# mattreturn1/ComputerVision_ObjectDetection_FeatureMatching

Hardware: AMD Instinct MI355X
Metric: matches+homographies/sec (10k x 10k SIFT, 50k RANSAC iters) at 1/2/4/8 GPUs (higher is better)
Workload: dtype i8-MFMA exact-int distances (i32 acc), fp64 DLT/Jacobi, fp32 reprojection; 1 GPU; c4: one global batch of 256 scenes x 1 model set, 10000x10000 descriptors, maxIters 50000, scenes sharded over 1 GPU(s) (256 on rank 0); problems_per_gpu=256, global_batch=256, parallelism=dp1, batches_in_flight=16, dist_backend=nccl, hw_queues=24

## Files before the change

computervision_objectdetection_featurematching_amd/csrc/api.cpp:

```cpp
#include <hip/hip_runtime.h>

#include <algorithm>
#include <cfloat>
#include <climits>
#include <cmath>
#include <cstdarg>
#include <cstdio>
#include <cstdlib>
#include <cstring>
#include <map>
#include <mutex>
#include <string>
#include <vector>

#include "../../include/mim.h"
#include "../../include/mim_detect.hpp"
#include "knn_coll.h"
#include "mim_internal.h"
#include "radius.h"

namespace mim {
void launch_prep_batch(const PrepJob* jobs, int njobs, int total_tiles, hipStream_t st);
void launch_knn(const ProbDev* probs, const KnnWork* works, int n_works, const int* seg_start, int n_blocks, Top2* parts,
                int* dyn_ctr, float kappa, float flip_ratio, hipStream_t st);
// ... 134 lines not shown
            if (p[i]) (void)hipHostFree(p[i]);
            if (ev[i]) (void)hipEventDestroy(ev[i]);
            p[i] = nullptr;
            ev[i] = nullptr;
        }
    }
};

template <class T> size_t vec_bytes(const std::vector<T>& v) { return sizeof(T) * v.size(); }

struct StageWriter {
    PinnedStage& ps;
    hipStream_t s;
    char* p = nullptr;
    size_t off = 0;
    hipError_t err;
    StageWriter(PinnedStage& ps_, size_t total, hipStream_t s_) : ps(ps_), s(s_) { err = ps.acquire(total, &p); }
    void put(void* dst, const void* a, size_t ab, const void* b = nullptr, size_t bb = 0) {
        if (err != hipSuccess || ab + bb == 0) return;
        if (ab) memcpy(p + off, a, ab);
        if (bb) memcpy(p + off + ab, b, bb);
        err = hipMemcpyAsync(dst, p + off, ab + bb, hipMemcpyHostToDevice, s);
        off += ab + bb;
    }
    template <class T> void put(const DevBuf& dst, const std::vector<T>& v) { put(dst.p, v.data(), vec_bytes(v)); }
    hipError_t done() { return err != hipSuccess ? err : ps.release_after(s); }
};

}

namespace mim {
struct RansacWs {
    DevBuf state, samples, hyp, counts, bounds, flags, irr_bits, irr, irr_cnt, cls, cls_tab, pass_bits, defer, defer_n, chains, best_h, cand, ncand, cex, cH, decided, stream,
        scratch, inl, tiles, tbox, perm, surv, nsurv, err;
    long long stream_len = 0;
};
}

struct mim_ctx {
    int device = 0;
    hipStream_t own = nullptr, stream = nullptr;
    std::mutex mu;
    std::string err;
    Arena arena;
    std::vector<SetRec> sets;
    DevBuf probs, works, parts, good_q, good_t, pts, n_good, results, masks, knn_idx, knn_dist, inl_tab, inl_out, knn_ctr, ham_works, flt_works;
    RansacWs rws;
    std::vector<ProbDev> h_probs;
    int n_ham_works = 0;
    int n_flt_works = 0;
    DevBuf ham_cross_works, colmin, cross_tab;
    int n_ham_cross_works = 0;
    long long n_colmin = 0;
    DevBuf topk_parts, topk_ham_works, topk_flt_works, topk_probs;
    int topk_splits = 0;
    DevBuf coll_parts, coll_ham_works, coll_flt_works, coll_i8_probs, coll_i8_works, coll_tab, coll_queries;
    int coll_groups = 0;
    int coll_i8_splits = 0;
    DevBuf rad_counts, rad_cursor, rad_offsets, rad_meta, rad_keys, rad_scratch, rad_ham_works, rad_flt_works, rad_i8_works,
        rad_probs;
    struct RadLast {
        bool valid = false;
        std::vector<mim_problem> problems;
        float r = 0.f;
        long long gen = -1;
        long long n_queries = 0, total = 0, longest = 0;
        int n_ham = 0, n_flt = 0, n_i8_works = 0, n_i8_blocks = 0;
// ... 105 lines not shown
    }
    c->stream = c->own;
    c->cur = c->own;
    const char* ex = getenv("MIM_RANSAC_EXACT");
    c->exact_all = (ex && ex[0] == '1') ? 1 : 0;
    const char* cc = getenv("MIM_CAND_CAP");
    c->cand_cap = cc ? std::max(1, atoi(cc)) : 0;
    const char* rc = getenv("MIM_ATTEMPT_REP_CAP");
    c->rep_cap = rc ? std::max(1, atoi(rc)) : 0;
    const char* sd = getenv("MIM_STREAM_DRAWS");
    c->stream_draws = sd ? std::max(4096LL, atoll(sd)) : 0;
    *out = c;
    return MIM_OK;
}

void mim_ctx_destroy(mim_ctx* c) {
    if (!c) return;
    (void)hipSetDevice(c->device);
    (void)hipStreamSynchronize(c->stream);
    for (auto& e : c->evs) (void)hipEventDestroy(e.e);
    for (hipEvent_t e : c->ev_pool) (void)hipEventDestroy(e);
    if (c->samp) (void)hipStreamSynchronize(c->samp);
    if (c->ev_samp_fork) (void)hipEventDestroy(c->ev_samp_fork);
    for (auto e : c->ev_samp)
        if (e) (void)hipEventDestroy(e);
    if (c->samp) (void)hipStreamDestroy(c->samp);
    mim::sift_ws_destroy(c->sift);
    for (mim::SiftWs* w : c->sift_scales) mim::sift_ws_destroy(w);
    c->stage.destroy();
    c->prep_stage.destroy();
    c->arena.release();
    for (DevBuf* b : {&c->probs, &c->works, &c->parts, &c->good_q, &c->good_t, &c->pts, &c->n_good,
                      &c->results, &c->masks, &c->knn_idx, &c->knn_dist, &c->inl_tab, &c->inl_out, &c->knn_ctr, &c->ham_works, &c->flt_works, &c->ham_cross_works, &c->colmin, &c->cross_tab, &c->topk_parts, &c->topk_ham_works, &c->topk_flt_works, &c->topk_probs, &c->coll_parts, &c->coll_ham_works, &c->coll_flt_works, &c->coll_i8_probs, &c->coll_i8_works, &c->coll_tab, &c->coll_queries, &c->rad_counts, &c->rad_cursor, &c->rad_offsets, &c->rad_meta, &c->rad_keys, &c->rad_scratch, &c->rad_ham_works, &c->rad_flt_works, &c->rad_i8_works, &c->rad_probs, &c->rws.state, &c->rws.samples,
                      &c->rws.hyp, &c->rws.counts, &c->rws.bounds, &c->rws.flags, &c->rws.irr_bits, &c->rws.irr, &c->rws.irr_cnt, &c->rws.cls, &c->rws.cls_tab, &c->rws.pass_bits, &c->rws.defer, &c->rws.defer_n, &c->rws.chains, &c->rws.best_h, &c->rws.cand, &c->rws.ncand, &c->rws.cex, &c->rws.cH, &c->rws.decided, &c->rws.stream, &c->rws.scratch, &c->rws.inl, &c->rws.tiles, &c->rws.tbox, &c->rws.perm, &c->rws.surv, &c->rws.nsurv, &c->rws.err, &c->prep_jobs})
        b->release();
    if (c->own) (void)hipStreamDestroy(c->own);
    delete c;
}

const char* mim_last_error(const mim_ctx* c) { return c ? c->err.c_str() : "null ctx"; }

mim_status mim_ctx_set_stream(mim_ctx* c, void* stream) {
    if (!c) return MIM_EINVAL;
    std::lock_guard<std::mutex> lk(c->mu);
    c->stream = stream ? (hipStream_t)stream : c->own;
    return MIM_OK;
}

mim_status mim_ctx_set_sampler_stream(mim_ctx* c, int32_t on) {
    if (!c) return MIM_EINVAL;
    std::lock_guard<std::mutex> lk(c->mu);
    c->samp_on = on != 0;
    return MIM_OK;
}

void* mim_ctx_get_stream(const mim_ctx* c) { return c ? (void*)c->stream : nullptr; }

mim_status mim_synchronize(mim_ctx* c) {
    if (!c) return MIM_EINVAL;
    HIPCHK(c, hipSetDevice(c->device));
    HIPCHK(c, hipStreamSynchronize(c->stream));
    return MIM_OK;
}

mim_status mim_set_timing(mim_ctx* c, int32_t enable) {
    if (!c) return MIM_EINVAL;
    c->timing = enable != 0;
// ... 1517 lines not shown
    }
    HIPCHK(c, c->rws.state.ensure(sizeof(RansacState) * std::max(n, 1)));
    HIPCHK(c, c->rws.samples.ensure(sizeof(int4) * it_total));
    HIPCHK(c, c->rws.hyp.ensure(sizeof(float) * 8 * it_total));
    HIPCHK(c, c->rws.counts.ensure(sizeof(int) * it_total));
    HIPCHK(c, c->rws.bounds.ensure(sizeof(int2) * it_total));
    const long long chunk_max = std::min<long long>(max_iters, 1 << 18);
    flag_per = (chunk_max * 28 + 4096 + 63) & ~63LL;
    const long long flag_cap = (long long)std::max(n, 1) * flag_per;
    HIPCHK(c, c->rws.flags.ensure((size_t)flag_cap));
    HIPCHK(c, c->rws.irr_bits.ensure((size_t)flag_cap / 8));
    const int irr_blocks = (int)((flag_per + kIrrBlock - 1) / kIrrBlock);
    HIPCHK(c, c->rws.irr.ensure(sizeof(int) * (size_t)std::max(n, 1) * irr_blocks * kIrrCap));
    HIPCHK(c, c->rws.irr_cnt.ensure(sizeof(int) * (size_t)std::max(n, 1) * irr_blocks));
    HIPCHK(c, c->rws.cls.ensure(sizeof(SamplerClass) * (size_t)std::max(n, 1)));
    HIPCHK(c, c->rws.cls_tab.ensure(sizeof(SamplerClassSlot) * ((size_t)q_max + 1)));
    HIPCHK(c, c->rws.pass_bits.ensure((size_t)flag_cap / 8));
    const int def_rounds = (int)((flag_per / 4 + 2 * kRansacDefRoundAttempts) / kRansacDefRoundAttempts);
    HIPCHK(c, c->rws.defer.ensure(sizeof(int2) * kRansacDefSlots * (size_t)std::max(n, 1) * def_rounds));
    HIPCHK(c, c->rws.defer_n.ensure(sizeof(int) * (size_t)std::max(n, 1) * def_rounds));
    HIPCHK(c, c->rws.chains.ensure(ransac_chain_bytes() * (size_t)std::max(n, 1)));
    HIPCHK(c, c->rws.best_h.ensure(sizeof(double) * 9 * std::max(n, 1)));
    const size_t cap = (size_t)std::max(n, 1) * 2 * kCandPerProblem;
    HIPCHK(c, c->rws.cand.ensure(sizeof(int) * cap));
    HIPCHK(c, c->rws.ncand.ensure(sizeof(int) * 2 * std::max(n, 1)));
    HIPCHK(c, c->rws.cex.ensure(sizeof(int) * cap));
    HIPCHK(c, c->rws.cH.ensure(sizeof(double) * 9 * cap));
    HIPCHK(c, c->rws.decided.ensure(sizeof(int) * cap));
    HIPCHK(c, c->rws.inl.ensure(sizeof(float4) * good_total));
    HIPCHK(c, c->rws.tiles.ensure(sizeof(uint4) * 128 * ((good_total + 31) / 32)));
    HIPCHK(c, c->rws.tbox.ensure(sizeof(float4) * ((good_total + 31) / 32)));
    HIPCHK(c, c->rws.perm.ensure(sizeof(int) * 2 * good_total));
    HIPCHK(c, c->rws.surv.ensure(sizeof(int) * it_total));
    HIPCHK(c, c->rws.nsurv.ensure(sizeof(int) * std::max(n, 1)));
    HIPCHK(c, c->rws.err.ensure(sizeof(int) * 4));
    HIPCHK(c, c->results.ensure(sizeof(mim_result) * std::max(n, 1)));
    HIPCHK(c, c->masks.ensure(good_total));
    HIPCHK(c, hipMemsetAsync(c->rws.err.p, 0, sizeof(int) * 4, c->stream));
    b = RansacBufs{};
    b.state = c->rws.state.as<RansacState>();
    b.samples = c->rws.samples.as<int4>();
    b.hyp = c->rws.hyp.as<float>();
    b.counts = c->rws.counts.as<int>();
    b.bounds = c->rws.bounds.as<int2>();
    b.flags = c->rws.flags.as<uint8_t>();
    b.irr_bits = c->rws.irr_bits.as<uint8_t>();
    b.best_h = c->rws.best_h.as<double>();
    b.cand = c->rws.cand.as<int>();
    b.ncand = c->rws.ncand.as<int>();
    b.cex = c->rws.cex.as<int>();
    b.cH = c->rws.cH.as<double>();
    b.decided = c->rws.decided.as<int>();
    b.flag_cap = flag_cap;
    b.irr = c->rws.irr.as<int>();
    b.irr_cnt = c->rws.irr_cnt.as<int>();
    b.pass_bits = c->rws.pass_bits.as<uint32_t>();
    b.defer = c->rws.defer.as<int2>();
    b.defer_n = c->rws.defer_n.as<int>();
    const char* cde = getenv("MIM_CHECK_DEFER");
    b.def_rounds = (cde && cde[0] == '0') ? 0 : def_rounds;
    b.irr_blocks = irr_blocks;
    b.cls = c->rws.cls.as<SamplerClass>();
    b.cls_tab = c->rws.cls_tab.as<SamplerClassSlot>();
    b.cls_tab_n = q_max + 1;
    b.chains = c->rws.chains.p;
    b.stream = c->rws.stream.as<uint32_t>();
    b.stream_len = c->rws.stream_len;
    b.inl = c->rws.inl.as<float4>();
    b.tiles = c->rws.tiles.as<uint4>();
    b.tbox = c->rws.tbox.as<float4>();
    b.perm = c->rws.perm.as<int>();
    b.surv = c->rws.surv.as<int>();
    b.nsurv = c->rws.nsurv.as<int>();
    b.err = c->rws.err.as<int>();
    if (c->samp_on < 0) {
        const char* e = getenv("MIM_SAMPLER_STREAM");
        c->samp_on = (e && e[0] == '0') ? 0 : 1;
    }
    if (c->samp_on && !c->samp) {
        HIPCHK(c, hipStreamCreateWithFlags(&c->samp, hipStreamNonBlocking));
        HIPCHK(c, hipEventCreateWithFlags(&c->ev_samp_fork, hipEventDisableTiming));
        for (auto& e : c->ev_samp) HIPCHK(c, hipEventCreateWithFlags(&e, hipEventDisableTiming));
    }
    b.s2 = c->samp_on ? c->samp : nullptr;
    b.ev_fork = c->ev_samp_fork;
    b.ev_samp[0] = c->ev_samp[0];
    b.ev_samp[1] = c->ev_samp[1];
    rp = RansacParams{};
    rp.thresh = prm->ransac_thresh > 0 ? prm->ransac_thresh : 3.0;
    rp.conf = prm->confidence;
    rp.max_iters = max_iters;
    rp.ratio = prm->ratio;
    rp.min_good = prm->min_good;
    rp.min_inliers = prm->min_inliers;
    rp.det_lo = prm->det_lo;
    rp.det_hi = prm->det_hi;
    rp.cand_cap = c->cand_cap;
    rp.rep_cap = c->rep_cap;
    return MIM_OK;
}

static mim_status ransac_enqueue_range(mim_ctx* c, int p0, int np, const RansacBufs& b, const RansacParams& rp,
                                       long long flag_per, int raw) {
    RansacBufs g = b;
    g.state += p0;
    g.flags += (long long)p0 * flag_per;
    g.irr_bits += (long long)p0 * flag_per / 8;
    g.flag_cap = (long long)np * flag_per;
    g.irr += (long long)p0 * b.irr_blocks * kIrrCap;
    g.irr_cnt += (long long)p0 * b.irr_blocks;
    g.cls += p0;
    g.pass_bits += (long long)p0 * flag_per / 32;
    g.defer += (long long)p0 * b.def_rounds * kRansacDefSlots;
    g.defer_n += (long long)p0 * b.def_rounds;
    g.chains = static_cast<char*>(b.chains) + (size_t)p0 * ransac_chain_bytes();
    g.best_h += 9LL * p0;
    g.cand += (long long)p0 * 2 * kCandPerProblem;
    g.ncand += 2 * p0;
    g.cex += (long long)p0 * 2 * kCandPerProblem;
    g.cH += 9LL * p0 * 2 * kCandPerProblem;
    g.decided += (long long)p0 * 2 * kCandPerProblem;
    g.nsurv += p0;
    ransac_enqueue(rp, np, c->probs.as<ProbDev>() + p0, c->pts.as<float4>(), c->n_good.as<int>() + p0, g,
                   c->masks.as<uint8_t>(), c->results.as<mim_result>() + p0, raw, c->cur, mark_cb, c, c->exact_all);
    HIPCHK(c, hipGetLastError());
    return MIM_OK;
}

static mim_status ransac_locked(mim_ctx* c, int n, const mim_params* prm, int raw) {
    RansacBufs b;
    RansacParams rp;
    long long flag_per = 0;
    mim_status s = ransac_prepare(c, n, prm, b, rp, flag_per);
    if (s != MIM_OK) return s;
    c->cur = c->stream;
    return ransac_enqueue_range(c, 0, n, b, rp, flag_per, raw);
}

static mim_status check_params(mim_ctx* c, const mim_params* p) {
    if (!p) return fail(c, MIM_EINVAL, "null params");
    if (!(p->confidence > 0 && p->confidence < 1)) return fail(c, MIM_EINVAL, "confidence must be in (0,1)");
    if (p->max_iters > 10000000) return fail(c, MIM_EINVAL, "max_iters too large");
    return MIM_OK;
}

extern "C" {

}

static mim_status batch_run_locked(mim_ctx* c, const mim_problem* problems, int32_t n, const mim_params* params,
                                   int filter) {
    HIPCHK(c, hipSetDevice(c->device));
    c->last_problems.assign(problems, problems + n);
    c->last_params = *params;
    c->last_filter = filter;
// ... 225 lines not shown
```

computervision_objectdetection_featurematching_amd/csrc/mim_internal.h:

```cpp
#pragma once
#include <hip/hip_runtime.h>
#include <stdint.h>

#include "knn_schedule.h"
#include "knn_topk_merge.h"

namespace mim {

constexpr int kDim = 128;
constexpr int kTileRows = 64;
constexpr int kTileBytes = kTileRows * kDim;
constexpr int kNormWords = 4 * kTileRows;
constexpr int kWave = 64;
#ifndef MIM_KNN_STAGE
#define MIM_KNN_STAGE 4
#endif
constexpr int kKnnStage = MIM_KNN_STAGE;

struct SetDev {
    const int8_t* frag;
    const int* norm;
    const float* f32;
    const float2* kp;
    int n;
// ... 155 lines not shown
    RansacState* state;
    int4* samples;
    float* hyp;
    int* counts;
    int2* bounds;
    double* best_h;
    int* cand;
    int* ncand;
    int* cex;
    double* cH;
    int* decided;
    uint8_t* flags;
    uint8_t* irr_bits;
    long long flag_cap;
    int* irr;
    int* irr_cnt;
    uint32_t* pass_bits;
    void* chains;
    int2* defer;
    int* defer_n;
    int def_rounds;
    int irr_blocks;
    SamplerClass* cls;
    SamplerClassSlot* cls_tab;
    int cls_tab_n;
    const uint32_t* stream;
    long long stream_len;
    float4* inl;
    uint4* tiles;
    float4* tbox;
    int* perm;
    int* surv;
    int* nsurv;
    int* err;
    hipStream_t s2;
    hipEvent_t ev_fork;
    hipEvent_t ev_samp[2];
};
}

#include <string>
#include <vector>
#include "../../include/mim.h"
namespace mim {
struct SiftWs;
SiftWs* sift_ws_create();
void sift_ws_destroy(SiftWs* w);
int sift_detect_compute(SiftWs* w, hipStream_t st, const uint8_t* img, int rows, int cols, long long step,
                        const uint8_t* mask, long long mstep, int max_kp, mim_keypoint* kps, float* desc, int* n_out,
                        std::string& err);
int sift_detect_compute_scales(std::vector<SiftWs*>& ws, hipStream_t st, const uint8_t* img, int rows, int cols,
                               long long step, int n_scales, const float* scales, int max_kp, mim_keypoint* kps,
                               float* desc, int* n_out, std::string& err);
int sift_resize_u8(SiftWs* w, hipStream_t st, const uint8_t* src, int rows, int cols, long long step, uint8_t* dst,
                   int drows, int dcols, double fx, double fy, std::string& err);
struct SiftDevOut {
    const mim_keypoint* kp;
    const float* desc;
    int n;
};
int sift_scales_device(std::vector<SiftWs*>& ws, hipStream_t st, const uint8_t* img, int rows, int cols,
                       long long step, int channels, int n_scales, const float* scales, SiftDevOut* out,
                       std::string& err);
int sift_bgr2gray_u8(SiftWs* w, hipStream_t st, const uint8_t* bgr, int rows, int cols, long long step, uint8_t* gray,
                     std::string& err);
int sift_copy_sets(const SiftDevOut* out, int n, float* const* ddesc, float2* const* dkp, hipStream_t st);
// ... 4 lines not shown
```

computervision_objectdetection_featurematching_amd/csrc/ransac.hip:

```cpp
#include <float.h>

#include <algorithm>
#include <climits>
#include <cstdio>
#include <cstdlib>
#include <vector>

#include "../../include/mim.h"
#include "mim_debug.h"
#include "mim_internal.h"

namespace mim {

__device__ __forceinline__ double d_hypot(double a, double b) {
    a = fabs(a);
    b = fabs(b);
    const bool ab = a > b;
    const double big = ab ? a : b, sm = ab ? b : a;
    const double r = sm / big;
    const double res = big * sqrt(1 + r * r);
    return (ab || b > 0) ? res : 0.0;
}

template <int n> __device__ __forceinline__ int pk(int i, int j) {
    static_assert(n <= 16, "packed index masks");
    return (int)(((unsigned)(i & 15) * (unsigned)((2 * n - 1 - i) & 31)) >> 1) + (j - i - 1);
}

template <int n> __device__ __forceinline__ int pk_any(int a, int b) {
    const int i = min(a, b), j = max(a, b);
    return pk<n>(i, j);
}

template <int n, int S>
__device__ void jacobi_fast(double* __restrict__ A, double* __restrict__ W, double* __restrict__ V,
                            double (&Ws)[n], int (&perm)[n]) {
#define AU(i, j) A[pk<n>((i), (j)) * S]
    const int trash = n * (n - 1) / 2 + n + n * n;
    const double eps = DBL_EPSILON;
// ... 2147 lines not shown
    if (rho < kScreenTight) eta = (float)eta_model;
    double Qs[9], Qd[9], Ai[9], H[9];
    square_to_quad(sx, sy, Qs);
    square_to_quad(dx, dy, Qd);
    Ai[0] = Qs[4] * Qs[8] - Qs[5] * Qs[7]; Ai[1] = Qs[2] * Qs[7] - Qs[1] * Qs[8]; Ai[2] = Qs[1] * Qs[5] - Qs[2] * Qs[4];
    Ai[3] = Qs[5] * Qs[6] - Qs[3] * Qs[8]; Ai[4] = Qs[0] * Qs[8] - Qs[2] * Qs[6]; Ai[5] = Qs[2] * Qs[3] - Qs[0] * Qs[5];
    Ai[6] = Qs[3] * Qs[7] - Qs[4] * Qs[6]; Ai[7] = Qs[1] * Qs[6] - Qs[0] * Qs[7]; Ai[8] = Qs[0] * Qs[4] - Qs[1] * Qs[3];
    mat3_mul(Qd, Ai, H);
    double hmax = 0;
#pragma unroll
    for (int i = 0; i < 9; ++i) hmax = fmax(hmax, fabs(H[i]));
    uncertain |= !(fabs(H[8]) > 1e-9 * hmax);
    const double inv = 1.0 / H[8];
#pragma unroll
    for (int i = 0; i < 8; ++i) Hd[i] = H[i] * inv;
#pragma unroll
    for (int i = 0; i < 8; ++i) uncertain |= !isfinite((float)Hd[i]);
}

typedef _Float16 h8v __attribute__((ext_vector_type(8)));
typedef float f16acc __attribute__((ext_vector_type(16)));
constexpr float kMfmaErr = 0x1p-15f;
constexpr float kPointScale = 0x1p15f;
constexpr double kHypScale = 0x1p15;
constexpr double kOutScale = 0x1p30;
#ifndef MIM_BOUND_CHUNK
#define MIM_BOUND_CHUNK 8
#endif
#ifndef MIM_BOUND_WAVES
#define MIM_BOUND_WAVES 4
#endif
constexpr int kBoundThreads = 64 * MIM_BOUND_WAVES;
constexpr int kSurvBlocks = 4;
constexpr int kTileChunk = MIM_BOUND_CHUNK;

__device__ __forceinline__ float clamp01(float x) { return __builtin_amdgcn_fmed3f(x, 0.f, 1.f); }

__device__ __forceinline__ void split_f16(float a, _Float16& hi, _Float16& lo) {
    asm volatile("" : "+v"(a));
    hi = (_Float16)a;
    lo = (_Float16)(a - (float)hi);
}
__device__ __forceinline__ void split_f16(double a, _Float16& hi, _Float16& lo) {
    float af = (float)a;
    asm volatile("" : "+v"(af));
    hi = (_Float16)af;
    lo = (_Float16)(float)(a - (double)(float)hi);
}

constexpr int kTileXBins = 1024;
constexpr int kTileYBins = 64;
constexpr int kTileStripsMax = 32;
constexpr int kTileKeys = kTileStripsMax * kTileYBins;
constexpr int kCapMinN = 128;

__global__ __launch_bounds__(256) void ransac_tiles_kernel(RansacState* __restrict__ st,
                                                           const ProbDev* __restrict__ probs,
                                                           const float4* __restrict__ pts,
                                                           uint4* __restrict__ tiles, float4* __restrict__ tbox,
                                                           int* __restrict__ perm, int* __restrict__ nsurv) {
    __shared__ float red[7][4];
    __shared__ int start[kTileKeys + 1], cur[kTileKeys];
    __shared__ unsigned char strip_of[kTileXBins];
    __shared__ int wred[4];
    const int p = blockIdx.x, tid = threadIdx.x;
    RansacState* Sp = st + p;
    if (tid == 0) nsurv[p] = 0;
    if (!Sp->active || Sp->done) return;
    const int n = Sp->n;
    const long long go = probs[p].good_off;
    const float4* __restrict__ P = pts + go;
    float mxy = 0.f, muv = 0.f, ms = 0.f;
    float x0 = INFINITY, x1 = -INFINITY, y0 = INFINITY, y1 = -INFINITY;
    for (int i = tid; i < n; i += 256) {
        const float4 q = P[i];
        mxy = fmaxf(mxy, fmaxf(fabsf(q.x), fabsf(q.y)));
        muv = fmaxf(muv, fmaxf(fabsf(q.z), fabsf(q.w)));
        ms = fmaxf(ms, fabsf(q.x) + fabsf(q.y) + fabsf(q.z) + fabsf(q.w));
        x0 = fminf(x0, q.x); x1 = fmaxf(x1, q.x);
        y0 = fminf(y0, q.y); y1 = fmaxf(y1, q.y);
    }
    for (int off = 32; off >= 1; off >>= 1) {
        mxy = fmaxf(mxy, __shfl_xor(mxy, off));
        muv = fmaxf(muv, __shfl_xor(muv, off));
        ms = fmaxf(ms, __shfl_xor(ms, off));
        x0 = fminf(x0, __shfl_xor(x0, off)); x1 = fmaxf(x1, __shfl_xor(x1, off));
        y0 = fminf(y0, __shfl_xor(y0, off)); y1 = fmaxf(y1, __shfl_xor(y1, off));
    }
    if ((tid & 63) == 0) {
        red[0][tid >> 6] = mxy;
        red[1][tid >> 6] = muv;
        red[2][tid >> 6] = ms;
        red[3][tid >> 6] = x0; red[4][tid >> 6] = x1;
        red[5][tid >> 6] = y0; red[6][tid >> 6] = y1;
    }
    __syncthreads();
    mxy = fmaxf(fmaxf(red[0][0], red[0][1]), fmaxf(red[0][2], red[0][3]));
    muv = fmaxf(fmaxf(red[1][0], red[1][1]), fmaxf(red[1][2], red[1][3]));
    ms = fmaxf(fmaxf(red[2][0], red[2][1]), fmaxf(red[2][2], red[2][3]));
    x0 = fminf(fminf(red[3][0], red[3][1]), fminf(red[3][2], red[3][3]));
// ... 105 lines not shown
        float bx0 = INFINITY, bx1 = -INFINITY, by0 = INFINITY, by1 = -INFINITY;
        if (row < n) {
            const float4 q = P[B[row]];
            bx0 = bx1 = q.x * sa;
            by0 = by1 = q.y * sa;
        }
#pragma unroll
        for (int off = 16; off >= 1; off >>= 1) {
            bx0 = fminf(bx0, __shfl_xor(bx0, off)); bx1 = fmaxf(bx1, __shfl_xor(bx1, off));
            by0 = fminf(by0, __shfl_xor(by0, off)); by1 = fmaxf(by1, __shfl_xor(by1, off));
        }
        if (t < nt && (tid & 31) == 0) {
            const float cx = 0.5f * (bx0 + bx1), cy = 0.5f * (by0 + by1);
            const float rx = fmaxf(bx1 - cx, cx - bx0) * (1.f + 0x1p-22f);
            const float ry = fmaxf(by1 - cy, cy - by0) * (1.f + 0x1p-22f);
            TB[t] = make_float4(cx, cy, rx, ry);
        }
    }
}

enum { kBoundUp = 0, kBoundLoUp = 1, kBoundCap = 2 };

template <int kMode, bool kList>
__global__ __launch_bounds__(kBoundThreads) void ransac_bound_mfma_kernel(const RansacState* __restrict__ st,
                                                                const ProbDev* __restrict__ probs,
                                                                const float4* __restrict__ pts,
                                                                const int4* __restrict__ samples,
                                                                const uint32_t* __restrict__ stream,
                                                                const uint4* __restrict__ tiles,
                                                                int2* __restrict__ bounds, int c0, int c1, int bpp,
                                                                float thr2, int n_probs,
                                                                const float4* __restrict__ tbox,
                                                                int* __restrict__ surv, int* __restrict__ nsurv,
                                                                int list_all) {
    constexpr bool kLo = kMode == kBoundLoUp;
    constexpr bool kCap = kMode == kBoundCap;
    static_assert(!(kList && kMode != kBoundUp), "the survivor list takes the full upper form");
    __shared__ uint4 lt[2][kTileChunk * 128];
    const int xcd = blockIdx.x & 7, j = blockIdx.x >> 3;
    const int p = xcd + 8 * (j / bpp), kb = j % bpp;
    if (p >= n_probs) return;
    const int tid = threadIdx.x, lane = tid & 63;
    const RansacState S = st[p];
    if (!S.active || S.done) return;
    if (kCap && !list_all && S.n < kCapMinN) {
        if (kb == 0 && tid == 0) nsurv[p] = -1;
        return;
    }
    const int n_list0 = kList ? nsurv[p] : 0;
    const bool contig = kList && n_list0 < 0;
    const int n_list = contig ? max(0, min(c1, S.produced) - c0) : n_list0;
    for (int lk = kb * kBoundThreads; !kList || lk < n_list; lk += bpp * kBoundThreads) {
    int it = c0 + kb * kBoundThreads + tid;
    bool act;
    if (kList) {
        act = lk + tid < n_list;
        it = !act ? c0 : contig ? c0 + lk + tid : surv[probs[p].it_off + lk + tid];
    } else {
        if (c0 + kb * kBoundThreads >= min(c1, S.produced)) return;
        act = it < c1 && it < S.produced;
    }
    const long long o = probs[p].it_off + it;
    const long long go = probs[p].good_off;
    const float4* __restrict__ P = pts + go;
    const int n = S.n;
    bool uncertain = false, invalid = false;
    float eta = 0.f;
    double Hd[8] = {0, 0, 0, 0, 0, 0, 0, 0};
    double eta_model = 0;
    if (act) {
        const int4 s4 = decode_sample(samples[o], stream, (unsigned)n, S.modM);
        bound_hypothesis(P, s4, Hd, invalid, uncertain, eta, eta_model);
    }
    const double isa = ldexp(1.0, -ilogb((double)S.sa)), rs = (double)S.sb * isa;
    double h[9] = {Hd[0] * rs, Hd[1] * rs, Hd[2] * S.sb, Hd[3] * rs, Hd[4] * rs, Hd[5] * S.sb,
                   Hd[6] * isa, Hd[7] * isa, 1.0};
    double hm = 0;
#pragma unroll
    for (int i = 0; i < 9; ++i) hm = fmax(hm, fabs(h[i]));
    int e = 0;
    (void)frexp(hm, &e);
    uncertain |= e > 24;
// ... 128 lines not shown
            const f16acc ex1 = __builtin_amdgcn_mfma_f32_32x32x16_f16(ax, b1x, zc, 0, 0, 0);
            const f16acc ey1 = __builtin_amdgcn_mfma_f32_32x32x16_f16(ay, b1y, zc, 0, 0, 0);
            const f16acc w1 = __builtin_amdgcn_mfma_f32_32x32x16_f16(ax, b1w, zc, 0, 0, 0);
#pragma unroll
            for (int r = 0; r < 16; ++r) {
                if (kLo) {
                    const float s0 = fabsf(ex0[r]) + fabsf(ey0[r]);
                    const float s1 = fabsf(ex1[r]) + fabsf(ey1[r]);
                    keep0 += clamp01(fmaf(C0, fabsf(w0[r]), E0) - s0);
                    keep1 += clamp01(fmaf(C1, fabsf(w1[r]), E1) - s1);
                    in0 += clamp01(fmaf(CL0, fabsf(w0[r]), EL0) - s0);
                    in1 += clamp01(fmaf(CL1, fabsf(w1[r]), EL1) - s1);
                } else {
                    keep0 += clamp01((fmaf(C0, fabsf(w0[r]), E0) - fabsf(ex0[r])) - fabsf(ey0[r]));
                    keep1 += clamp01((fmaf(C1, fabsf(w1[r]), E1) - fabsf(ex1[r])) - fabsf(ey1[r]));
                }
            }
          }
        }
        asm volatile("s_waitcnt vmcnt(0)" ::: "memory");
        __syncthreads();
    }
    const float k0 = keep0 + __shfl_xor(keep0, 32), k1 = keep1 + __shfl_xor(keep1, 32);
    const double m2 = 0x1p-24 * 1.25 * (double)(16 * nt + 2);
    const double kk = (double)(lowh ? k0 : k1);
    const int hi = min(n, max(0, (int)floor(kk + m2 * (kk + 1.0)) - (32 * nt - n)));
    int lo = 0;
    if (kLo) {
        const float i0 = in0 + __shfl_xor(in0, 32), i1 = in1 + __shfl_xor(in1, 32);
        const double ii = (double)(lowh ? i0 : i1);
        lo = min(hi, max(0, (int)ceil(ii - m2 * (ii + 1.0))));
    }
    if (act) bounds[o] = invalid ? make_int2(-1, -1) : (uncertain ? make_int2(0, n) : make_int2(lo, hi));
    if (kCap) {
        const bool on = count && (list_all || hi > max(3, max(S.max_good, S.lo_max)));
        const unsigned long long m = __ballot(on);
        if (m) {
            int base = 0;
            if (lane == __ffsll((long long)m) - 1) base = atomicAdd(nsurv + p, __popcll(m));
            base = __shfl(base, __ffsll((long long)m) - 1);
            if (on) surv[probs[p].it_off + base + __popcll(m & ((1ull << lane) - 1))] = it;
        }
    }
    if (!kList) break;
    }
}

__device__ int exact_count(const float4* __restrict__ P, int n, int4 s4, double* D, float thr2, double (&H)[9]) {
    const float4 a = P[s4.x], b = P[s4.y], c = P[s4.z], d = P[s4.w];
    const float M[8] = {a.x, a.y, b.x, b.y, c.x, c.y, d.x, d.y};
    const float m[8] = {a.z, a.w, b.z, b.w, c.z, c.w, d.z, d.w};
    if (!run_kernel4<64>(M, m, D, H)) return -1;
    float Hf[8];
#pragma unroll
    for (int i = 0; i < 8; ++i) Hf[i] = (float)H[i];
    int cnt = 0;
    for (int i = 0; i < n; ++i) {
        const float4 q = P[i];
        cnt += reproj_err(Hf, q.x, q.y, q.z, q.w) <= thr2;
    }
    return cnt;
}

__global__ __launch_bounds__(64) void ransac_bound_check_kernel(const RansacState* __restrict__ st,
                                                                const ProbDev* __restrict__ probs,
                                                                const float4* __restrict__ pts,
                                                                const int4* __restrict__ samples,
                                                                const uint32_t* __restrict__ stream,
                                                                const int2* __restrict__ bounds, int c0, int c1,
                                                                int bpp, float thr2, unsigned long long* stats) {
    __shared__ double sd[kJ9D * 64];
    const int p = blockIdx.x / bpp, lane = threadIdx.x;
// ... 1055 lines not shown

__global__ __launch_bounds__(256) void rng_stream_kernel(const unsigned long long* __restrict__ seg_state,
                                                         uint32_t* __restrict__ out, long long len, int seg,
                                                         int n_seg) {
    const int i = blockIdx.x * blockDim.x + threadIdx.x;
    if (i >= n_seg) return;
    unsigned long long st = seg_state[i];
    const long long p0 = (long long)i * seg;
    const int m = (int)min((long long)seg, len - p0);
    for (int k = 0; k < m; ++k) {
        out[p0 + k] = (uint32_t)st;
        st = (unsigned long long)(uint32_t)st * 4164903690ull + (st >> 32);
    }
}

void launch_rng_stream(const unsigned long long* seg_state, uint32_t* out, long long len, int seg, int n_seg,
                       hipStream_t s) {
    rng_stream_kernel<<<(n_seg + 255) / 256, 256, 0, s>>>(seg_state, out, len, seg, n_seg);
}

void ransac_enqueue(const RansacParams& prm, int n_probs, const ProbDev* probs, const float4* pts,
                    const int* n_good, const RansacBufs& b, uint8_t* masks, mim_result* results, int raw,
                    hipStream_t s, void (*mark)(void*, const char*, hipStream_t), void* mark_ctx, int exact_all) {
    if (n_probs <= 0) return;
    ransac_init_kernel<<<(n_probs + 255) / 256, 256, 0, s>>>(b.state, n_good, n_probs, prm.max_iters, prm.min_good,
                                                             b.best_h);
    const int max_iters = prm.max_iters > 1 ? prm.max_iters : 1;
    const char* sw = getenv("MIM_SAMPLER_WALK");
    const int use_chain = !(sw && sw[0] == '1');
    int first = max_iters <= 4096 ? 512 : 4096;
    if (const char* fc = getenv("MIM_FIRST_CHUNK")) first = std::max(1, atoi(fc));
    int c0 = 0, chunk = first;
    const float thr2 = (float)(prm.thresh * prm.thresh);
    if (!exact_all) ransac_tiles_kernel<<<n_probs, 256, 0, s>>>(b.state, probs, pts, b.tiles, b.tbox, b.perm, b.nsurv);
    const char* bce = getenv("MIM_BOUND_CAP");
    const int bound_cap = (bce && bce[0] == '0') ? 0 : 1;
    const char* bae = getenv("MIM_BOUND_CAP_ALL");
    const int cap_all = (bae && bae[0] == '1') ? 1 : 0;
    const bool split = b.s2 && !exact_all;
    hipStream_t ss = split ? b.s2 : s;
    if (split) {
        (void)hipEventRecord(b.ev_fork, s);
        (void)hipStreamWaitEvent(ss, b.ev_fork, 0);
        mark(mark_ctx, "fork", ss);
    }
    int ci = 0, c1_first = 0;
    const int cap = prm.cand_cap > 0 ? std::min(prm.cand_cap, kCandCap) : kCandCap;
    const char* pe = getenv("MIM_PRESCREEN");
    const int prescreen = (pe && pe[0] == '0') ? 0 : 1;
    const char* se = getenv("MIM_SETTLE");
    const int settle = (se && se[0] == '0') ? 0 : 1;
    const char* we = getenv("MIM_WINNER_H");
    const int winner_h = !we ? 2 : we[0] == '1' ? 1 : we[0] == '0' ? 0 : 2;
    int min_blocks = kSamplerMinBlocks;
    if (const char* mb = getenv("MIM_SAMPLER_MIN_BLOCKS")) min_blocks = std::max(0, atoi(mb));
    const char* she = getenv("MIM_SAMPLER_SHARE");
    const int share = (she && she[0] == '0') ? 0 : 1;
    const char* spe = getenv("MIM_SHARE_SPREAD");
    while (c0 < max_iters) {
        const int c1 = (int)std::min<long long>((long long)c0 + chunk, max_iters);
        const int wcap = (int)(std::min<long long>((long long)(c1 - c0) * 28 + 4096, b.flag_cap / std::max(n_probs, 1)) & ~63LL);
        const int west = (int)std::min<long long>(wcap, (long long)(c1 - c0) * kAttemptRateEst + 4096);
        const int bppw_cap = std::max(1, wcap / kAttemptSpan);
        const int bppw = (std::max((west + kAttemptSpan - 1) / kAttemptSpan,
                                   std::min(bppw_cap, (min_blocks + n_probs - 1) / n_probs)) + 7) / 8 * 8;
        const int rep_cap = prm.rep_cap > 0 ? std::min(prm.rep_cap, kAttemptRepCap) : kAttemptRepCap;
        const int spread = std::min(spe ? std::max(0, atoi(spe)) : wcap / 16, wcap / 2);
        const bool dbg_ncls = getenv("MIM_DEBUG_NCLASS") != nullptr;
        if (dbg_ncls && split) (void)hipStreamSynchronize(s);
        ransac_class_kernel<<<1, kClassThreads, 0, ss>>>(b.state, n_probs, c1, wcap, share, spread, b.cls_tab,
                                                         b.cls_tab_n, b.cls);
// ... 39 lines not shown
        ransac_small_kernel<<<n_probs, kSmallThreads, 0, ss>>>(b.state, probs, pts, b.stream, b.stream_len, b.samples,
                                                              c1, b.err);
        ransac_sample_kernel<<<n_probs, 64, 0, ss>>>(b.state, probs, pts, b.stream, b.stream_len, b.samples, c1, b.err,
                                                    b.flags, b.irr_bits, wcap, b.cls);
        mark(mark_ctx, "sample", ss);
        if (split) {
            (void)hipEventRecord(b.ev_samp[ci & 1], ss);
            (void)hipStreamWaitEvent(s, b.ev_samp[ci & 1], 0);
            mark(mark_ctx, "join", s);
        }
        ++ci;
        const int bpp256 = (c1 - c0 + 255) / 256;
        const int bppb = (c1 - c0 + kBoundThreads - 1) / kBoundThreads;
        if (exact_all) {
            const int bpp64 = (c1 - c0 + 63) / 64;
            ransac_hypo_kernel<<<n_probs * bpp64, 64, 0, s>>>(b.state, probs, pts, b.samples, b.stream, b.hyp, b.counts, c0, c1,
                                                             bpp64);
            mark(mark_ctx, "hypo", s);
            ransac_score_kernel<<<n_probs * bpp256, 256, 0, s>>>(b.state, probs, pts, b.hyp, b.counts, c0, c1,
                                                                bpp256, thr2);
            mark(mark_ctx, "score", s);
            ransac_select_kernel<<<n_probs, 64, 0, s>>>(b.state, probs, b.counts, c1, prm.conf);
            mark(mark_ctx, "select", s);
            if (getenv("MIM_DEBUG_TRACE") && n_probs == 1) {
                std::vector<int> hc(c1 - c0);
                std::vector<int4> hs(c1 - c0);
                (void)hipMemcpyAsync(hc.data(), b.counts + c0, sizeof(int) * (c1 - c0), hipMemcpyDeviceToHost, s);
                (void)hipMemcpyAsync(hs.data(), b.samples + c0, sizeof(int4) * (c1 - c0), hipMemcpyDeviceToHost, s);
                (void)hipStreamSynchronize(s);
                for (int i = 0; i < c1 - c0; ++i)
                    fprintf(stderr, "[trace] %d %d %d %d %d %d\n", c0 + i, hc[i], hs[i].x, hs[i].y, hs[i].z, hs[i].w);
            }
        } else {
            if (c0 == 0)
                ransac_bound_mfma_kernel<kBoundLoUp, false><<<8 * ((n_probs + 7) / 8) * bppb, kBoundThreads, 0, s>>>(
                    b.state, probs, pts, b.samples, b.stream, b.tiles, b.bounds, c0, c1, bppb, thr2, n_probs, b.tbox,
                    b.surv, b.nsurv, 0);
            else if (!bound_cap)
                ransac_bound_mfma_kernel<kBoundUp, false><<<8 * ((n_probs + 7) / 8) * bppb, kBoundThreads, 0, s>>>(
                    b.state, probs, pts, b.samples, b.stream, b.tiles, b.bounds, c0, c1, bppb, thr2, n_probs, b.tbox,
                    b.surv, b.nsurv, 0);
            else {
                const int bppl = std::min(bppb, kSurvBlocks);
                ransac_bound_mfma_kernel<kBoundCap, false><<<8 * ((n_probs + 7) / 8) * bppb, kBoundThreads, 0, s>>>(
                    b.state, probs, pts, b.samples, b.stream, b.tiles, b.bounds, c0, c1, bppb, thr2, n_probs, b.tbox,
                    b.surv, b.nsurv, cap_all);
                ransac_bound_mfma_kernel<kBoundUp, true><<<8 * ((n_probs + 7) / 8) * bppl, kBoundThreads, 0, s>>>(
                    b.state, probs, pts, b.samples, b.stream, b.tiles, b.bounds, c0, c1, bppl, thr2, n_probs, b.tbox,
                    b.surv, b.nsurv, 0);
                if (getenv("MIM_DEBUG_NSURV")) {
                    std::vector<int> h(n_probs);
                    (void)hipMemcpyAsync(h.data(), b.nsurv, sizeof(int) * n_probs, hipMemcpyDeviceToHost, s);
                    (void)hipStreamSynchronize(s);
                    long long sum = 0; int mx = 0, small = 0;
                    for (int i = 0; i < n_probs; ++i) {
                        sum += std::max(h[i], 0);
                        mx = std::max(mx, h[i]);
                        small += h[i] < 0;
                    }
                    fprintf(stderr, "[mim] chunk [%d,%d): survivors mean %.1f max %d (%d small problems on the full bound alone)\n",
                            c0, c1, (double)sum / n_probs, mx, small);
                }
            }
            mark(mark_ctx, "score", s);
            if (getenv("MIM_CHECK_BOUNDS")) {
                unsigned long long* dst = nullptr;
                unsigned long long h[6] = {0, 0, 0, 0, 0, 0};
                if (hipMalloc(&dst, sizeof h) == hipSuccess) {
                    (void)hipMemsetAsync(dst, 0, sizeof h, s);
                    const int bpp64 = (c1 - c0 + 63) / 64;
                    ransac_bound_check_kernel<<<n_probs * bpp64, 64, 0, s>>>(b.state, probs, pts, b.samples, b.stream,
                                                                             b.bounds, c0, c1, bpp64, thr2, dst);
                    (void)hipMemcpyAsync(h, dst, sizeof h, hipMemcpyDeviceToHost, s);
                    (void)hipStreamSynchronize(s);
                    (void)hipFree(dst);
                }
                fprintf(stderr, "[mim] bound check chunk [%d,%d): checked %llu lo_viol %llu hi_viol %llu valid_mismatch %llu "
                        "mean_width %.2f tight %llu\n", c0, c1, h[0], h[1], h[2], h[3], h[0] ? (double)h[4] / h[0] : 0.0, h[5]);
            }
            const int L = c0 == 0 ? 0 : 1;
            ransac_cand_kernel<<<n_probs, kCandThreads, 0, s>>>(b.state, probs, b.bounds, c1, b.cand, b.ncand, L,
                                                                cap);
            if (prescreen) {
                ransac_prescreen_kernel<<<n_probs * kPreWaves, 64, 0, s>>>(b.state, probs, b.bounds, pts, b.samples,
                                                                          b.stream, b.cand, b.ncand, b.cex, b.cH,
                                                                          b.decided, thr2, L, cap);
                if (settle)
                    ransac_settle_kernel<<<n_probs, 64, 0, s>>>(b.state, probs, b.bounds, b.cand, b.ncand, b.cex, b.cH,
                                                                b.decided, L, cap, winner_h);
            }
            mark(mark_ctx, "cand", s);
            if (prescreen && getenv("MIM_CHECK_PRESCREEN")) {
                unsigned long long* dst = nullptr;
                unsigned long long h[2] = {0, 0};
                if (hipMalloc(&dst, sizeof h) == hipSuccess) {
                    (void)hipMemsetAsync(dst, 0, sizeof h, s);
// ... 56 lines not shown
```

Measured before the change: 38480 problems/s.

## Add pilot bound pass to seed survivor cap for first RANSAC chunk

In the first chunk, the change runs a small pilot of 256 iterations with the full lower and upper bound. It records the best lower bound per problem with a wave max and an atomicMax into a new pilot_lo buffer. The rest of the first chunk then goes through the cap/survivor cascade, with the pilot bar raising the threshold, so fewer hypotheses need the full exact bound. The survivor count buffer is now double-slotted so consecutive cascades can alternate. The cost is extra kernel launches and a heuristic gate based on block count and max_iters.

```diff
diff --git a/computervision_objectdetection_featurematching_amd/csrc/api.cpp b/computervision_objectdetection_featurematching_amd/csrc/api.cpp
--- a/computervision_objectdetection_featurematching_amd/csrc/api.cpp
+++ b/computervision_objectdetection_featurematching_amd/csrc/api.cpp
@@ -190,7 +190,7 @@
 namespace mim {
 struct RansacWs {
     DevBuf state, samples, hyp, counts, bounds, flags, irr_bits, irr, irr_cnt, cls, cls_tab, pass_bits, defer, defer_n, chains, best_h, cand, ncand, cex, cH, decided, stream,
-        scratch, inl, tiles, tbox, perm, surv, nsurv, err;
+        scratch, inl, tiles, tbox, perm, surv, nsurv, pilot_lo, err;
     long long stream_len = 0;
 };
 }
@@ -362,7 +362,7 @@
     c->arena.release();
     for (DevBuf* b : {&c->probs, &c->works, &c->parts, &c->good_q, &c->good_t, &c->pts, &c->n_good,
                       &c->results, &c->masks, &c->knn_idx, &c->knn_dist, &c->inl_tab, &c->inl_out, &c->knn_ctr, &c->ham_works, &c->flt_works, &c->ham_cross_works, &c->colmin, &c->cross_tab, &c->topk_parts, &c->topk_ham_works, &c->topk_flt_works, &c->topk_probs, &c->coll_parts, &c->coll_ham_works, &c->coll_flt_works, &c->coll_i8_probs, &c->coll_i8_works, &c->coll_tab, &c->coll_queries, &c->rad_counts, &c->rad_cursor, &c->rad_offsets, &c->rad_meta, &c->rad_keys, &c->rad_scratch, &c->rad_ham_works, &c->rad_flt_works, &c->rad_i8_works, &c->rad_probs, &c->rws.state, &c->rws.samples,
-                      &c->rws.hyp, &c->rws.counts, &c->rws.bounds, &c->rws.flags, &c->rws.irr_bits, &c->rws.irr, &c->rws.irr_cnt, &c->rws.cls, &c->rws.cls_tab, &c->rws.pass_bits, &c->rws.defer, &c->rws.defer_n, &c->rws.chains, &c->rws.best_h, &c->rws.cand, &c->rws.ncand, &c->rws.cex, &c->rws.cH, &c->rws.decided, &c->rws.stream, &c->rws.scratch, &c->rws.inl, &c->rws.tiles, &c->rws.tbox, &c->rws.perm, &c->rws.surv, &c->rws.nsurv, &c->rws.err, &c->prep_jobs})
+                      &c->rws.hyp, &c->rws.counts, &c->rws.bounds, &c->rws.flags, &c->rws.irr_bits, &c->rws.irr, &c->rws.irr_cnt, &c->rws.cls, &c->rws.cls_tab, &c->rws.pass_bits, &c->rws.defer, &c->rws.defer_n, &c->rws.chains, &c->rws.best_h, &c->rws.cand, &c->rws.ncand, &c->rws.cex, &c->rws.cH, &c->rws.decided, &c->rws.stream, &c->rws.scratch, &c->rws.inl, &c->rws.tiles, &c->rws.tbox, &c->rws.perm, &c->rws.surv, &c->rws.nsurv, &c->rws.pilot_lo, &c->rws.err, &c->prep_jobs})
         b->release();
     if (c->own) (void)hipStreamDestroy(c->own);
     delete c;
@@ -1946,7 +1946,8 @@
     HIPCHK(c, c->rws.tbox.ensure(sizeof(float4) * ((good_total + 31) / 32)));
     HIPCHK(c, c->rws.perm.ensure(sizeof(int) * 2 * good_total));
     HIPCHK(c, c->rws.surv.ensure(sizeof(int) * it_total));
-    HIPCHK(c, c->rws.nsurv.ensure(sizeof(int) * std::max(n, 1)));
+    HIPCHK(c, c->rws.nsurv.ensure(sizeof(int) * 2 * std::max(n, 1)));
+    HIPCHK(c, c->rws.pilot_lo.ensure(sizeof(int) * std::max(n, 1)));
     HIPCHK(c, c->rws.err.ensure(sizeof(int) * 4));
     HIPCHK(c, c->results.ensure(sizeof(mim_result) * std::max(n, 1)));
     HIPCHK(c, c->masks.ensure(good_total));
@@ -1986,6 +1987,7 @@
     b.perm = c->rws.perm.as<int>();
     b.surv = c->rws.surv.as<int>();
     b.nsurv = c->rws.nsurv.as<int>();
+    b.pilot_lo = c->rws.pilot_lo.as<int>();
     b.err = c->rws.err.as<int>();
     if (c->samp_on < 0) {
         const char* e = getenv("MIM_SAMPLER_STREAM");
@@ -2034,7 +2036,8 @@
     g.cex += (long long)p0 * 2 * kCandPerProblem;
     g.cH += 9LL * p0 * 2 * kCandPerProblem;
     g.decided += (long long)p0 * 2 * kCandPerProblem;
-    g.nsurv += p0;
+    g.nsurv += 2 * p0;
+    g.pilot_lo += p0;
     ransac_enqueue(rp, np, c->probs.as<ProbDev>() + p0, c->pts.as<float4>(), c->n_good.as<int>() + p0, g,
                    c->masks.as<uint8_t>(), c->results.as<mim_result>() + p0, raw, c->cur, mark_cb, c, c->exact_all);
     HIPCHK(c, hipGetLastError());
diff --git a/computervision_objectdetection_featurematching_amd/csrc/mim_internal.h b/computervision_objectdetection_featurematching_amd/csrc/mim_internal.h
--- a/computervision_objectdetection_featurematching_amd/csrc/mim_internal.h
+++ b/computervision_objectdetection_featurematching_amd/csrc/mim_internal.h
@@ -211,6 +211,7 @@
     int* perm;
     int* surv;
     int* nsurv;
+    int* pilot_lo;
     int* err;
     hipStream_t s2;
     hipEvent_t ev_fork;
diff --git a/computervision_objectdetection_featurematching_amd/csrc/ransac.hip b/computervision_objectdetection_featurematching_amd/csrc/ransac.hip
--- a/computervision_objectdetection_featurematching_amd/csrc/ransac.hip
+++ b/computervision_objectdetection_featurematching_amd/csrc/ransac.hip
@@ -5,6 +5,7 @@
 #include <cstdio>
 #include <cstdlib>
 #include <vector>
+#include <type_traits>
 
 #include "../../include/mim.h"
 #include "mim_debug.h"
@@ -2218,6 +2219,9 @@
 #endif
 constexpr int kBoundThreads = 64 * MIM_BOUND_WAVES;
 constexpr int kSurvBlocks = 4;
+constexpr int kPilotIters = 256;
+constexpr int kPilotCut = 1024;
+constexpr int kPilotMinBlocks = 2048;
 constexpr int kTileChunk = MIM_BOUND_CHUNK;
 
 __device__ __forceinline__ float clamp01(float x) { return __builtin_amdgcn_fmed3f(x, 0.f, 1.f); }
@@ -2244,14 +2248,18 @@
                                                            const ProbDev* __restrict__ probs,
                                                            const float4* __restrict__ pts,
                                                            uint4* __restrict__ tiles, float4* __restrict__ tbox,
-                                                           int* __restrict__ perm, int* __restrict__ nsurv) {
+                                                           int* __restrict__ perm, int* __restrict__ nsurv,
+                                                           int* __restrict__ pilot_lo) {
     __shared__ float red[7][4];
     __shared__ int start[kTileKeys + 1], cur[kTileKeys];
     __shared__ unsigned char strip_of[kTileXBins];
     __shared__ int wred[4];
     const int p = blockIdx.x, tid = threadIdx.x;
     RansacState* Sp = st + p;
-    if (tid == 0) nsurv[p] = 0;
+    if (tid == 0) {
+        nsurv[2 * p] = nsurv[2 * p + 1] = 0;
+        pilot_lo[p] = 0;
+    }
     if (!Sp->active || Sp->done) return;
     const int n = Sp->n;
     const long long go = probs[p].good_off;
@@ -2423,10 +2431,10 @@
                                                                 float thr2, int n_probs,
                                                                 const float4* __restrict__ tbox,
                                                                 int* __restrict__ surv, int* __restrict__ nsurv,
-                                                                int list_all) {
+                                                                int list_all, int slot, int* __restrict__ pilot_lo) {
     constexpr bool kLo = kMode == kBoundLoUp;
     constexpr bool kCap = kMode == kBoundCap;
-    static_assert(!(kList && kMode != kBoundUp), "the survivor list takes the full upper form");
+    static_assert(!(kList && kCap), "the survivor list takes a full form");
     __shared__ uint4 lt[2][kTileChunk * 128];
     const int xcd = blockIdx.x & 7, j = blockIdx.x >> 3;
     const int p = xcd + 8 * (j / bpp), kb = j % bpp;
@@ -2434,11 +2442,14 @@
     const int tid = threadIdx.x, lane = tid & 63;
     const RansacState S = st[p];
     if (!S.active || S.done) return;
+    nsurv += 2 * p + slot;
+    if (kCap && kb == 0 && tid == 0) nsurv[1 - 2 * slot] = 0;
     if (kCap && !list_all && S.n < kCapMinN) {
-        if (kb == 0 && tid == 0) nsurv[p] = -1;
+        if (kb == 0 && tid == 0) *nsurv = -1;
         return;
     }
-    const int n_list0 = kList ? nsurv[p] : 0;
+    const int bar = kCap ? max(3, max(max(S.max_good, S.lo_max), pilot_lo[p])) : 0;
+    const int n_list0 = kList ? *nsurv : 0;
     const bool contig = kList && n_list0 < 0;
     const int n_list = contig ? max(0, min(c1, S.produced) - c0) : n_list0;
     for (int lk = kb * kBoundThreads; !kList || lk < n_list; lk += bpp * kBoundThreads) {
@@ -2633,12 +2644,18 @@
         lo = min(hi, max(0, (int)ceil(ii - m2 * (ii + 1.0))));
     }
     if (act) bounds[o] = invalid ? make_int2(-1, -1) : (uncertain ? make_int2(0, n) : make_int2(lo, hi));
+    if (kLo && pilot_lo) {
+        int wl = count ? lo : 0;
+#pragma unroll
+        for (int off = 32; off >= 1; off >>= 1) wl = max(wl, __shfl_xor(wl, off));
+        if (lane == 0 && wl > 0) atomicMax(pilot_lo + p, wl);
+    }
     if (kCap) {
-        const bool on = count && (list_all || hi > max(3, max(S.max_good, S.lo_max)));
+        const bool on = count && (list_all || hi > bar);
         const unsigned long long m = __ballot(on);
         if (m) {
             int base = 0;
-            if (lane == __ffsll((long long)m) - 1) base = atomicAdd(nsurv + p, __popcll(m));
+            if (lane == __ffsll((long long)m) - 1) base = atomicAdd(nsurv, __popcll(m));
             base = __shfl(base, __ffsll((long long)m) - 1);
             if (on) surv[probs[p].it_off + base + __popcll(m & ((1ull << lane) - 1))] = it;
         }
@@ -3760,11 +3777,16 @@
     if (const char* fc = getenv("MIM_FIRST_CHUNK")) first = std::max(1, atoi(fc));
     int c0 = 0, chunk = first;
     const float thr2 = (float)(prm.thresh * prm.thresh);
-    if (!exact_all) ransac_tiles_kernel<<<n_probs, 256, 0, s>>>(b.state, probs, pts, b.tiles, b.tbox, b.perm, b.nsurv);
+    if (!exact_all)
+        ransac_tiles_kernel<<<n_probs, 256, 0, s>>>(b.state, probs, pts, b.tiles, b.tbox, b.perm, b.nsurv, b.pilot_lo);
     const char* bce = getenv("MIM_BOUND_CAP");
     const int bound_cap = (bce && bce[0] == '0') ? 0 : 1;
     const char* bae = getenv("MIM_BOUND_CAP_ALL");
     const int cap_all = (bae && bae[0] == '1') ? 1 : 0;
+    const char* bpe = getenv("MIM_BOUND_PILOT");
+    const long long first_blocks = (long long)n_probs * ((first + kBoundThreads - 1) / kBoundThreads);
+    const bool pilot = bound_cap && max_iters > 4096 && (bpe ? bpe[0] == '1' : first_blocks >= kPilotMinBlocks);
+    int cap_slot = 0;
     const bool split = b.s2 && !exact_all;
     hipStream_t ss = split ? b.s2 : s;
     if (split) {
@@ -3870,36 +3892,50 @@
                     fprintf(stderr, "[trace] %d %d %d %d %d %d\n", c0 + i, hc[i], hs[i].x, hs[i].y, hs[i].z, hs[i].w);
             }
         } else {
-            if (c0 == 0)
-                ransac_bound_mfma_kernel<kBoundLoUp, false><<<8 * ((n_probs + 7) / 8) * bppb, kBoundThreads, 0, s>>>(
-                    b.state, probs, pts, b.samples, b.stream, b.tiles, b.bounds, c0, c1, bppb, thr2, n_probs, b.tbox,
-                    b.surv, b.nsurv, 0);
-            else if (!bound_cap)
-                ransac_bound_mfma_kernel<kBoundUp, false><<<8 * ((n_probs + 7) / 8) * bppb, kBoundThreads, 0, s>>>(
-                    b.state, probs, pts, b.samples, b.stream, b.tiles, b.bounds, c0, c1, bppb, thr2, n_probs, b.tbox,
-                    b.surv, b.nsurv, 0);
-            else {
-                const int bppl = std::min(bppb, kSurvBlocks);
-                ransac_bound_mfma_kernel<kBoundCap, false><<<8 * ((n_probs + 7) / 8) * bppb, kBoundThreads, 0, s>>>(
-                    b.state, probs, pts, b.samples, b.stream, b.tiles, b.bounds, c0, c1, bppb, thr2, n_probs, b.tbox,
-                    b.surv, b.nsurv, cap_all);
-                ransac_bound_mfma_kernel<kBoundUp, true><<<8 * ((n_probs + 7) / 8) * bppl, kBoundThreads, 0, s>>>(
-                    b.state, probs, pts, b.samples, b.stream, b.tiles, b.bounds, c0, c1, bppl, thr2, n_probs, b.tbox,
-                    b.surv, b.nsurv, 0);
+            const int gx8 = 8 * ((n_probs + 7) / 8);
+            auto cascade = [&](auto full_mode, int a, int e, int* fold) {
+                constexpr int kFull = decltype(full_mode)::value;
+                const int bpa = (e - a + kBoundThreads - 1) / kBoundThreads, bppl = std::min(bpa, kSurvBlocks);
+                ransac_bound_mfma_kernel<kBoundCap, false><<<gx8 * bpa, kBoundThreads, 0, s>>>(
+                    b.state, probs, pts, b.samples, b.stream, b.tiles, b.bounds, a, e, bpa, thr2, n_probs, b.tbox,
+                    b.surv, b.nsurv, cap_all, cap_slot, b.pilot_lo);
+                ransac_bound_mfma_kernel<kFull, true><<<gx8 * bppl, kBoundThreads, 0, s>>>(
+                    b.state, probs, pts, b.samples, b.stream, b.tiles, b.bounds, a, e, bppl, thr2, n_probs, b.tbox,
+                    b.surv, b.nsurv, 0, cap_slot, fold);
                 if (getenv("MIM_DEBUG_NSURV")) {
-                    std::vector<int> h(n_probs);
-                    (void)hipMemcpyAsync(h.data(), b.nsurv, sizeof(int) * n_probs, hipMemcpyDeviceToHost, s);
+                    std::vector<int> h(2 * n_probs);
+                    (void)hipMemcpyAsync(h.data(), b.nsurv, sizeof(int) * 2 * n_probs, hipMemcpyDeviceToHost, s);
                     (void)hipStreamSynchronize(s);
                     long long sum = 0; int mx = 0, small = 0;
                     for (int i = 0; i < n_probs; ++i) {
-                        sum += std::max(h[i], 0);
-                        mx = std::max(mx, h[i]);
-                        small += h[i] < 0;
+                        const int v = h[2 * i + cap_slot];
+                        sum += std::max(v, 0);
+                        mx = std::max(mx, v);
+                        small += v < 0;
                     }
                     fprintf(stderr, "[mim] chunk [%d,%d): survivors mean %.1f max %d (%d small problems on the full bound alone)\n",
-                            c0, c1, (double)sum / n_probs, mx, small);
+                            a, e, (double)sum / n_probs, mx, small);
                 }
-            }
+                cap_slot ^= 1;
+            };
+            if (c0 == 0 && pilot && c1 > kPilotIters) {
+                constexpr int bpp0 = (kPilotIters + kBoundThreads - 1) / kBoundThreads;
+                ransac_bound_mfma_kernel<kBoundLoUp, false><<<gx8 * bpp0, kBoundThreads, 0, s>>>(
+                    b.state, probs, pts, b.samples, b.stream, b.tiles, b.bounds, 0, kPilotIters, bpp0, thr2, n_probs,
+                    b.tbox, b.surv, b.nsurv, 0, 0, b.pilot_lo);
+                const int cut = std::min(kPilotCut, c1);
+                cascade(std::integral_constant<int, kBoundLoUp>{}, kPilotIters, cut, b.pilot_lo);
+                if (cut < c1) cascade(std::integral_constant<int, kBoundLoUp>{}, cut, c1, b.pilot_lo);
+            } else if (c0 == 0)
+                ransac_bound_mfma_kernel<kBoundLoUp, false><<<gx8 * bppb, kBoundThreads, 0, s>>>(
+                    b.state, probs, pts, b.samples, b.stream, b.tiles, b.bounds, c0, c1, bppb, thr2, n_probs, b.tbox,
+                    b.surv, b.nsurv, 0, 0, nullptr);
+            else if (!bound_cap)
+                ransac_bound_mfma_kernel<kBoundUp, false><<<gx8 * bppb, kBoundThreads, 0, s>>>(
+                    b.state, probs, pts, b.samples, b.stream, b.tiles, b.bounds, c0, c1, bppb, thr2, n_probs, b.tbox,
+                    b.surv, b.nsurv, 0, 0, nullptr);
+            else
+                cascade(std::integral_constant<int, kBoundUp>{}, c0, c1, nullptr);
             mark(mark_ctx, "score", s);
             if (getenv("MIM_CHECK_BOUNDS")) {
                 unsigned long long* dst = nullptr;
```

Result: no change. 38470 problems/s (-0.0%).
